# qingpingmo/OCN

Measured on AMD Instinct MI355X. Metric: candidate-edges/sec (CN predictor fwd), ogbl-collab shape, higher is better.
Workload: dtype f32

## Files before the change

include/ocn_hip.h:

```cpp
#ifndef OCN_HIP_H
#define OCN_HIP_H

#include <stdint.h>

#ifdef __cplusplus
extern "C" {
#endif

#define OCN_ABI_VERSION 9
#define OCN_EINVAL (-1)
#define OCN_ECAP   (-2)

#define OCN_ST_CAP  1
#define OCN_ST_SCAN 2
#define OCN_SCAN_POISON (-1)

#define OCN_F_CN1 1u
#define OCN_F_CN2 2u

int ocn_abi_version(void);

int64_t ocn_scan_workspace_bytes(int64_t n);

int ocn_zero_regions(void* const* ptrs, const int64_t* bytes, int32_t n, void* stream);
// ... 170 lines not shown
int ocn_philox4x32(const uint32_t* ctr , uint32_t key0, uint32_t key1, int64_t n, uint32_t* out ,
                   void* stream);
int ocn_complement_count(const int64_t* rowptrK, const int32_t* colK, int64_t n_cols, int32_t* count ,
                         void* stream);
int32_t ocn_sample_stage_cols(void);
int ocn_sample_complement_rows(const int64_t* rowptrK, const int32_t* colK, int64_t n_cols, const int64_t* rows, int64_t Q,
                               int64_t per, int64_t q0, uint64_t seed, int64_t* out , void* stream);
int ocn_sample_complement_pairs(const int64_t* rowptrK, const int32_t* colK, int64_t n_cols,
                                const int64_t* cptr , int64_t T, int64_t t0, uint64_t seed,
                                int64_t* out , void* stream);

int64_t ocn_sample_two_hop_window_cols(void);
int ocn_sample_two_hop(const int64_t* rowptrA, const int32_t* colA, const int64_t* rowptrM, const int32_t* colM, int64_t n_cols,
                       const int64_t* rows, int64_t Q, int32_t drop_self, int64_t window_cols ,
                       const int64_t* sptr , const int64_t* sid , int64_t q0, uint64_t seed,
                       int32_t* count , int64_t* out , void* stream);

int ocn_gather_schedule(const int32_t* gcost, int64_t n_groups, int64_t segment, int32_t* perm, void* stream);

int ocn_cn_weights_cn6(uint64_t* histA, uint64_t* histB, int64_t N, const float* innerprod, int32_t* scalars,
                       float* nip_out, const float* s2_exact , const float* s3_exact ,
                       void* stream);
int ocn_cn_gather3(const int64_t* rowptrA, const int32_t* colA, const int64_t* src, const int64_t* dst,
                   const int64_t* order, int64_t B, const int64_t* off, const uint8_t* flagsA,
                   const uint8_t* flagsB, const float* weightsA, const float* weightsB, const float* nip,
                   const float* h, int32_t H, float* xcn1, float* xcn2, float* xcn3, float* xij, void* stream);

int ocn_cn3_flags(const int64_t* rowptrA, const int32_t* colA, const int64_t* rowptrT, const int32_t* colT,
                  const uint32_t* bitmapP, int64_t bm_stride_words, const int64_t* src, const int64_t* dst,
                  const int64_t* order , int64_t B, int64_t n_cols, const int64_t* off, uint8_t* flags,
                  int64_t flags_cap, uint64_t* hist , int32_t* cnt3, int32_t* status,
                  const int64_t* nds , const int64_t* chunk_off , void* stream);

int ocn_cn_gather3_backward(const int64_t* rowptrA, const int32_t* colA, const int64_t* src, const int64_t* dst,
                            const int64_t* order, int64_t B, const int64_t* off, const uint8_t* flagsA,
                            const uint8_t* flagsB, const float* weightsA, const float* weightsB, const float* nip,
                            const float* h, int32_t H, const float* g1, const float* g2, const float* g3,
                            const float* g4, float* dh, void* stream);

int ocn_cn_gather_backward(const int64_t* rowptrA, const int32_t* colA,
                           const int64_t* src, const int64_t* dst, const int64_t* order, int64_t B,
                           const int64_t* off, const uint8_t* flags, const int32_t* wc,
                           const float* weights, const float* h, int32_t H,
                           const float* g1, const float* g2, const float* g3, float* dh, void* stream);

int64_t ocn_cn_gather_backward_det_workspace_bytes(int64_t N, int64_t B, int64_t flags_cap);
int ocn_cn_gather_backward_det(const int64_t* rowptrA, const int32_t* colA, const int64_t* src, const int64_t* dst,
                               int64_t B, const int64_t* off, const uint8_t* flags, const int32_t* wc, int64_t flags_cap,
                               const float* weights, const float* h, int64_t N, int32_t H, const float* g1,
                               const float* g2, const float* g3, float* dh, void* workspace, void* stream);
int64_t ocn_cn_gather_backward_det_keys_offset(int64_t N);
int ocn_cn_gather_backward_det_lists(const int64_t* rowptrA, const int32_t* colA, const int64_t* src, const int64_t* dst,
                                     int64_t B, const int64_t* off, const uint8_t* flags, int64_t flags_cap, int64_t N,
                                     void* workspace, void* stream);

int ocn_spmm_csr(const int64_t* rowptr, const int32_t* col, const float* val, int64_t n_rows,
                 const float* x, int32_t F, const float* pre, const float* post,
                 int32_t mode, int32_t edge_scale, int32_t self_mode,
                 float* y, void* stream);

int ocn_spmm_csr_rows(const int64_t* rowptr, const int32_t* col, const float* val, int64_t n_rows,
                      const float* x, int32_t F, const float* pre, const float* post,
                      int32_t mode, int32_t edge_scale, int32_t self_mode,
                      const int64_t* rows, int64_t n_list, float* y, void* stream);

int ocn_spmm_csr_max_arg(const int64_t* rowptr, const int32_t* col, const float* val, int64_t n_rows,
                         const float* x, int32_t F, float* y, int32_t* arg, void* stream);
int ocn_spmm_max_backward(const int64_t* rowptrT, const int32_t* colT, const float* valT, int64_t n_rows,
                          const int32_t* arg, const float* g, int32_t F, float* gx, void* stream);

int ocn_deg_rsqrt(const int64_t* rowptr, const float* val, int64_t n_rows, float add, float* out,
                  void* stream);

int64_t ocn_spgemm_max_cols(void);
int ocn_spgemm_pattern_count(const int64_t* rowptrA, const int32_t* colA, int64_t n_rows,
                             const int64_t* rowptrB, const int32_t* colB, int64_t n_colsB,
                             int32_t* row_count, uint32_t* bitmap ,
                             int64_t bm_stride_words, void* stream);
int ocn_spgemm_pattern_fill(const int64_t* rowptrA, const int32_t* colA, int64_t n_rows,
                            const int64_t* rowptrB, const int32_t* colB, int64_t n_colsB,
                            const int64_t* rowptrC, int32_t* colC, void* stream);
int32_t ocn_cn_flags_small_graph_cols(void);
int64_t ocn_cn_flags_pair_min_batch(int64_t min_rows);
int ocn_spgemm_bit_rows(const int64_t* rowptrA, const int32_t* colA, int64_t n_rows, const int64_t* rowptrB, const int32_t* colB,
                        int64_t n_colsB, const int64_t* rows, int64_t n_req, int32_t* done, uint32_t* bitmap,
                        int64_t bm_stride_words, void* stream);

int ocn_dense_from_csr(const int64_t* rowptr, const int32_t* col, int64_t n, int64_t ld, int8_t* dense, int8_t* denseT,
                       void* stream);
int ocn_dense_block_mm_bits(const int8_t* A, const int8_t* Bt, int64_t ld, int64_t K, int32_t r0, int32_t r1, int32_t c0,
                            int32_t c1, int32_t fold, uint32_t* bits, int64_t bm_stride_words, void* stream);
int ocn_bitrows_from_csr(const int64_t* rowptr, const int32_t* col, int64_t n_rows, uint32_t* bits, int64_t bm_stride_words,
                         void* stream);
int ocn_bitrows_count(const uint32_t* bits, int64_t bm_stride_words, int64_t n_rows, int64_t n_cols, int32_t* row_count,
                      void* stream);
int ocn_bitrows_fill(const uint32_t* bits, int64_t bm_stride_words, int64_t n_rows, int64_t n_cols, const int64_t* rowptr,
                     int32_t* col, void* stream);

int ocn_csr_union_count(const int64_t* rowptrA, const int32_t* colA, const int64_t* rowptrB, const int32_t* colB,
                        int64_t n_rows, int32_t* count, void* stream);
int ocn_csr_union_fill(const int64_t* rowptrA, const int32_t* colA, const int64_t* rowptrB, const int32_t* colB,
                       int64_t n_rows, const int64_t* rowptrC , int32_t* colC, void* stream);
int64_t ocn_bitrows_insert_workspace_bytes(int64_t nnzD);
int ocn_bitrows_insert(const int64_t* rowptrA, const int32_t* colA, const int64_t* rowptrT, const int32_t* colT,
                       const int64_t* rowptrD, const int32_t* colD, int64_t n, int64_t nnzD, uint32_t* bits,
                       int64_t bm_stride_words, int32_t* added, void* workspace, void* stream);

int ocn_csr_minus_count(const int64_t* rowptrA, const int32_t* colA, const int64_t* rowptrB, const int32_t* colB,
                        int64_t n_rows, int32_t* count, void* stream);
int ocn_csr_minus_fill(const int64_t* rowptrA, const int32_t* colA, const int64_t* rowptrB, const int32_t* colB,
                       int64_t n_rows, const int64_t* rowptrC , int32_t* colC, void* stream);
int64_t ocn_bitrows_remove_workspace_bytes(int64_t nnzD);
int ocn_bitrows_remove(const int64_t* rowptrA0, const int32_t* colA0, const int64_t* rowptrT0, const int32_t* colT0,
                       const int64_t* rowptrA, const int32_t* colA, const int64_t* rowptrT, const int32_t* colT,
                       const int64_t* rowptrD, const int32_t* colD, int64_t n, int64_t nnzD, uint32_t* bits,
                       int64_t bm_stride_words, int32_t* removed, void* workspace, void* stream);

int64_t ocn_rows_neighbourhood_workspace_bytes(int64_t n_list);
int ocn_rows_neighbourhood(const int64_t* rowptrT, const int32_t* colT, int64_t n, const int64_t* rows, int64_t n_list,
                           uint32_t* bits, void* workspace, void* stream);
int ocn_bitlist_count(const uint32_t* bits, int64_t n_bits, int32_t* count, void* stream);
int ocn_bitlist_fill(const uint32_t* bits, int64_t n_bits, const int64_t* off , int64_t* out,
                     void* stream);

int ocn_rows_ln_relu(const float* x, const float* gamma, const float* beta, float eps, int32_t relu,
                     int64_t rows, int32_t H, float* y, void* stream);
int ocn_combine3(const float* coef, const float* x1, const float* x2, const float* x3, int64_t n,
                 float* out, void* stream);

int ocn_fill_rows(float* dst, int64_t ld, int32_t n_cols, const float* vec, const int64_t* row_range,
                  int64_t max_rows, void* stream);

typedef struct OcnLinearGroup {
  const float* X; int64_t ldX;
  int64_t M;
  const void* Wp;
  const float* bias;
  const float* gamma; const float* beta; float eps;
  int32_t relu;
  const float* scale;
  const float* addend; int64_t ldAdd;
  const float* dotw; const float* dotb;
  float* Y; int64_t ldY;
  const int64_t* row_range;
  const int64_t* y_row_map;
  int32_t add_bcast;
} OcnLinearGroup;

int64_t ocn_linear_panel_bytes(int32_t N, int32_t K);
int ocn_linear_split_weight(const float* W, int32_t N, int32_t K, void* Wp, void* stream);
int ocn_linear_bf16x6(const float* X, int64_t M, int32_t K, const void* Wp, int32_t N,
                      const float* bias, const float* gamma, const float* beta, float eps,
                      int32_t relu, const float* dotw, const float* dotb, float* Y, void* stream);
int ocn_linear_grouped(const OcnLinearGroup* groups, int32_t n_groups, int32_t K, int32_t N, void* stream);

typedef struct OcnHeadsArgs {
  const float* x[3];
  int64_t ldx, B;
  int32_t H;
  const void* p_first[3];
  const void* p_mid[2];
  const void* p_out[3];
  const float* vec;
  const int64_t* ranges;
  const int64_t* y_row_map;
  float* y;
// ... 42 lines not shown
```

ocn_amd/_lib.py:

```python
from __future__ import annotations

import ctypes
import glob
import os
import subprocess
from ctypes import c_float, c_int32, c_int64, c_void_p

_HERE = os.path.dirname(os.path.abspath(__file__))
_ROOT = os.path.dirname(_HERE)
LIB_PATH = os.environ.get("OCN_LIB_PATH", os.path.join(_HERE, "libocn_hip.so"))
CSRC = os.path.join(_HERE, "csrc")
INCLUDE = os.path.join(_ROOT, "include")

_P = c_void_p
ABI_VERSION = 9
SIGNATURES = {
    "ocn_abi_version": (c_int32, []),
    "ocn_scan_workspace_bytes": (c_int64, [c_int64]),
    "ocn_zero_regions": (c_int32, [_P, _P, c_int32, _P]),
    "ocn_check_edges": (c_int32, [_P, _P, c_int64, c_int64, c_int64, _P, _P]),
    "ocn_edge_offsets": (c_int32, [_P, _P, c_int64, _P, _P, _P]),
    "ocn_class_order": (c_int32, [_P, _P, _P, c_int64, _P, _P, _P, _P, _P, _P]),
    "ocn_scan_i32": (c_int32, [_P, c_int64, _P, _P, _P]),
    "ocn_order_workspace_bytes": (c_int64, [c_int64]),
    "ocn_order_by_node": (c_int32, [_P, c_int64, c_int64, _P, _P, _P]),
    "ocn_order_by_node_finish": (c_int32, [_P, c_int64, c_int64, _P, _P, _P]),
    "ocn_order_by_node_finish_rec": (c_int32, [_P, _P, _P, _P, c_int64, c_int64, _P, _P, _P, _P]),
    "ocn_batch_prep": (c_int32, [_P, _P, c_int64, _P, _P, c_int64, _P, _P, _P, c_int32, _P]),
    "ocn_cn_flags": (c_int32, [_P, _P, _P, _P, _P, _P, _P, c_int64, _P, c_int64, _P, _P, _P, c_int64, c_int64, _P, _P, c_int64, _P,
                               _P, _P, _P, _P, _P, _P]),
    "ocn_cn_flags_rec": (c_int32, [_P, _P, _P, _P, _P, _P, _P, c_int64, _P, c_int64, _P, _P, _P, c_int64, c_int64, _P, _P, c_int64, _P,
                                   _P, _P, _P, _P, _P, _P]),
    "ocn_chunk_offsets": (c_int32, [_P, _P, _P, _P, c_int64, _P, _P, _P]),
    "ocn_walk_chunk": (c_int32, []),
    "ocn_cn_walk_flags": (c_int32, [_P, _P, _P, _P, _P, _P, c_int64, _P, _P, _P, c_int64, _P, _P, c_int64, _P, _P, _P,
                                    _P, _P]),
    "ocn_neighbor_degree_sum": (c_int32, [_P, _P, c_int64, _P, _P]),
    "ocn_walk_prep_max_batch": (c_int32, []),
    "ocn_cn_flags_small_graph_cols": (c_int32, []),
    "ocn_cn_flags_pair_min_batch": (c_int64, [c_int64]),
    "ocn_walk_prep": (c_int32, [_P, _P, _P, _P, c_int64, c_int32, _P, _P, _P, _P, _P, _P, _P, _P, _P, _P, _P, _P, _P]),
    "ocn_cn_walk_group": (c_int32, [_P, _P, _P, _P, _P, c_int64, _P, _P, _P, _P, _P, _P, _P, c_int64, _P, _P, _P, _P]),
    "ocn_walk_rev_offsets": (c_int32, [_P, _P, _P, _P, _P, c_int64, _P, _P, _P]),
    "ocn_cn_weights_cn5": (c_int32, [_P, c_int64, _P, _P, c_int32, _P, _P]),
    "ocn_cn5_column_stats": (c_int32, [_P, c_int64, _P, _P]),
    "ocn_cn_colsum_workspace_bytes": (c_int64, [c_int64, c_int64]),
    "ocn_cn_colsum_exact": (c_int32, [_P, _P, _P, c_int64, _P, _P, _P, _P, c_int64, _P, c_int64, _P, _P, _P, _P, _P, _P, _P]),
    "ocn_cn_weights_cn7": (c_int32, [_P, c_int64, c_float, _P, _P, _P]),
    "ocn_cn_gather": (c_int32, [_P, _P, _P, _P, _P, c_int64, _P, _P, _P, _P, _P, c_int32, c_int64, _P, _P, _P, _P, _P,
                                _P, _P, _P, _P, _P]),
    "ocn_cn8_pool": (c_int32, [_P, _P, _P, _P, _P, _P, _P, c_int64, _P, c_int64, _P, _P, _P, c_int64, c_int64, _P, c_int32, _P, _P,
                               _P, _P, _P, _P]),
    "ocn_cn_pool_frozen": (c_int32, [_P, _P, _P, _P, _P, _P, _P, c_int64, _P, c_int64, _P, _P, _P, c_int64, c_int64, _P, _P, c_int32, _P,
                                     _P, _P, _P, _P, _P]),
    "ocn_cn_attribution": (c_int32, [_P, _P, _P, _P, c_int64, _P, _P, _P, c_int64, _P, _P, c_int32, _P, _P, _P, _P, _P]),
    "ocn_cn_node_sums": (c_int32, [_P, _P, _P, _P, _P, _P, _P, c_int64, _P, c_int64, _P, _P, _P, c_int64, c_int64, _P, _P, _P, _P, _P,
                                   _P, _P]),
    "ocn_row_diff_stage_cols": (c_int32, []),
    "ocn_row_diff_count": (c_int32, [_P, _P, _P, _P, _P, c_int64, c_int32, _P, _P]),
    "ocn_row_diff_fill": (c_int32, [_P, _P, _P, _P, _P, c_int64, c_int32, _P, _P, _P]),
    "ocn_two_hop_window_cols": (c_int64, []),
    "ocn_two_hop_diff_count": (c_int32, [_P, _P, _P, _P, c_int64, _P, c_int64, c_int32, c_int64, _P, _P]),
    "ocn_two_hop_diff_fill": (c_int32, [_P, _P, _P, _P, c_int64, _P, c_int64, c_int32, c_int64, _P, _P, _P]),
    "ocn_two_hop_sums_window_cols": (c_int64, []),
    "ocn_two_hop_sums_fill": (c_int32, [_P, _P, _P, _P, c_int64, _P, c_int64, c_int32, c_int64, _P, c_int32, _P, _P, _P, _P]),
    "ocn_frontier_window_cols": (c_int64, []),
    "ocn_frontier_count": (c_int32, [_P, _P, _P, _P, c_int64, _P, c_int64, c_int32, c_int64, _P, _P, _P, _P, _P, _P]),
    "ocn_frontier_sums_fill": (c_int32, [_P, _P, _P, _P, c_int64, _P, c_int64, c_int32, c_int64, _P, _P, _P, _P, _P, _P, _P, _P, _P,
                                         _P]),
    "ocn_segment_topk_max_k": (c_int32, []),
    "ocn_segment_topk": (c_int32, [_P, _P, c_int64, c_int32, _P, _P, _P]),
    "ocn_segment_rank": (c_int32, [_P, _P, _P, c_int64, _P, _P, c_int64, _P, _P, _P]),
    "ocn_philox4x32": (c_int32, [_P, ctypes.c_uint32, ctypes.c_uint32, c_int64, _P, _P]),
    "ocn_complement_count": (c_int32, [_P, _P, c_int64, _P, _P]),
    "ocn_sample_stage_cols": (c_int32, []),
    "ocn_sample_complement_rows": (c_int32, [_P, _P, c_int64, _P, c_int64, c_int64, c_int64, ctypes.c_uint64, _P, _P]),
    "ocn_sample_complement_pairs": (c_int32, [_P, _P, c_int64, _P, c_int64, c_int64, ctypes.c_uint64, _P, _P]),
    "ocn_sample_two_hop_window_cols": (c_int64, []),
    "ocn_sample_two_hop": (c_int32, [_P, _P, _P, _P, c_int64, _P, c_int64, c_int32, c_int64, _P, _P, c_int64, ctypes.c_uint64, _P, _P,
                                     _P]),
    "ocn_gather_schedule": (c_int32, [_P, c_int64, c_int64, _P, _P]),
    "ocn_coo_to_csr_workspace_bytes": (c_int64, [c_int64, c_int64, c_int32, c_int32]),
    "ocn_coo_to_csr": (c_int32, [_P, _P, c_int64, c_int64, c_int64, c_int32, c_int32, _P, _P, _P, _P, _P]),
    "ocn_wgrad_workspace_bytes": (c_int64, [c_int64, c_int32, c_int32]),
    "ocn_wgrad": (c_int32, [_P, c_int64, _P, c_int64, c_int64, c_int32, c_int32, _P, _P, _P, _P]),
    "ocn_cn_weights_cn6": (c_int32, [_P, _P, c_int64, _P, _P, _P, _P, _P, _P]),
    "ocn_cn_gather3": (c_int32, [_P, _P, _P, _P, _P, c_int64, _P, _P, _P, _P, _P, _P, _P, c_int32, _P, _P, _P, _P, _P]),
    "ocn_cn3_flags": (c_int32, [_P, _P, _P, _P, _P, c_int64, _P, _P, _P, c_int64, c_int64, _P, _P, c_int64, _P, _P, _P, _P, _P, _P]),
    "ocn_cn_gather3_backward": (c_int32, [_P, _P, _P, _P, _P, c_int64, _P, _P, _P, _P, _P, _P, _P, c_int32, _P, _P, _P, _P, _P, _P]),
    "ocn_cn_gather_backward": (c_int32, [_P, _P, _P, _P, _P, c_int64, _P, _P, _P, _P, _P, c_int32, _P, _P, _P, _P, _P]),
    "ocn_cn_gather_backward_det_workspace_bytes": (c_int64, [c_int64, c_int64, c_int64]),
    "ocn_cn_gather_backward_det": (c_int32, [_P, _P, _P, _P, c_int64, _P, _P, _P, c_int64, _P, _P, c_int64, c_int32, _P, _P, _P, _P,
                                             _P, _P]),
    "ocn_cn_gather_backward_det_keys_offset": (c_int64, [c_int64]),
    "ocn_cn_gather_backward_det_lists": (c_int32, [_P, _P, _P, _P, c_int64, _P, _P, c_int64, c_int64, _P, _P]),
    "ocn_ln_drop_relu_workspace_bytes": (c_int64, [c_int32]),
    "ocn_ln_drop_relu_forward": (c_int32, [_P, _P, _P, c_float, c_float, ctypes.c_uint64, c_int32, c_int64, c_int32, _P, _P, _P]),
    "ocn_ln_drop_relu_backward": (c_int32, [_P, _P, _P, _P, _P, c_float, ctypes.c_uint64, c_int32, c_int64, c_int32, _P, _P, _P, _P, _P]),
    "ocn_dropout_keep_mask": (c_int32, [ctypes.c_uint64, c_float, c_int64, _P, _P]),
    "ocn_mix3_workspace_bytes": (c_int64, []),
    "ocn_mix3_backward": (c_int32, [_P, _P, _P, _P, _P, c_int64, _P, _P, _P, _P, _P, _P]),
    "ocn_spmm_csr": (c_int32, [_P, _P, _P, c_int64, _P, c_int32, _P, _P, c_int32, c_int32, c_int32, _P, _P]),
    "ocn_spmm_csr_rows": (c_int32, [_P, _P, _P, c_int64, _P, c_int32, _P, _P, c_int32, c_int32, c_int32, _P, c_int64, _P, _P]),
    "ocn_spmm_csr_max_arg": (c_int32, [_P, _P, _P, c_int64, _P, c_int32, _P, _P, _P]),
    "ocn_spmm_max_backward": (c_int32, [_P, _P, _P, c_int64, _P, _P, c_int32, _P, _P]),
    "ocn_deg_rsqrt": (c_int32, [_P, _P, c_int64, c_float, _P, _P]),
    "ocn_spgemm_max_cols": (c_int64, []),
    "ocn_spgemm_pattern_count": (c_int32, [_P, _P, c_int64, _P, _P, c_int64, _P, _P, c_int64, _P]),
    "ocn_spgemm_pattern_fill": (c_int32, [_P, _P, c_int64, _P, _P, c_int64, _P, _P, _P]),
    "ocn_spgemm_bit_rows": (c_int32, [_P, _P, c_int64, _P, _P, c_int64, _P, c_int64, _P, _P, c_int64, _P]),
    "ocn_dense_from_csr": (c_int32, [_P, _P, c_int64, c_int64, _P, _P, _P]),
    "ocn_dense_block_mm_bits": (c_int32, [_P, _P, c_int64, c_int64, c_int32, c_int32, c_int32, c_int32, c_int32, _P, c_int64, _P]),
    "ocn_bitrows_from_csr": (c_int32, [_P, _P, c_int64, _P, c_int64, _P]),
    "ocn_bitrows_count": (c_int32, [_P, c_int64, c_int64, c_int64, _P, _P]),
    "ocn_bitrows_fill": (c_int32, [_P, c_int64, c_int64, c_int64, _P, _P, _P]),
    "ocn_csr_union_count": (c_int32, [_P, _P, _P, _P, c_int64, _P, _P]),
    "ocn_csr_union_fill": (c_int32, [_P, _P, _P, _P, c_int64, _P, _P, _P]),
    "ocn_bitrows_insert_workspace_bytes": (c_int64, [c_int64]),
    "ocn_bitrows_insert": (c_int32, [_P, _P, _P, _P, _P, _P, c_int64, c_int64, _P, c_int64, _P, _P, _P]),
    "ocn_csr_minus_count": (c_int32, [_P, _P, _P, _P, c_int64, _P, _P]),
    "ocn_csr_minus_fill": (c_int32, [_P, _P, _P, _P, c_int64, _P, _P, _P]),
    "ocn_bitrows_remove_workspace_bytes": (c_int64, [c_int64]),
    "ocn_bitrows_remove": (c_int32, [_P, _P, _P, _P, _P, _P, _P, _P, _P, _P, c_int64, c_int64, _P, c_int64, _P, _P, _P]),
# ... 124 lines not shown
```

ocn_amd/csrc/cn_flags.hip:

```cpp
#include "common.h"


__device__ __forceinline__ bool sampled_has(const int32_t* samp, const int32_t* __restrict__ row, i64 n,
                                            int32_t key) {
  int lo = 0, hi = OCN_WAVE;
  while (lo < hi) {
    const int mid = (lo + hi) >> 1;
    if (samp[mid] <= key) lo = mid + 1; else hi = mid;
  }
  if (lo == 0) return false;
  const int s = lo - 1;
  const i64 p0 = ((i64)s * n) >> 6, p1 = ((i64)(s + 1) * n) >> 6;
  return sorted_has(row + p0, p1 - p0, key);
}

#define T1_CAP 1024

#define LH_MAX_COLS 8192

__device__ __forceinline__ i64 wave_uniform(i64 v) {
  const unsigned lo = __builtin_amdgcn_readfirstlane((unsigned)(u64)v), hi = __builtin_amdgcn_readfirstlane((unsigned)((u64)v >> 32));
  return (i64)(((u64)hi << 32) | lo);
}
__device__ __forceinline__ bool lanes_have(int32_t t, int32_t key) {
  int pos = 0;
#pragma unroll
  for (int step = OCN_WAVE / 2; step > 0; step >>= 1)
    if (__shfl(t, pos + step - 1, OCN_WAVE) < key) pos += step;
  return __shfl(t, pos, OCN_WAVE) == key;
}

template <bool HAS_T2, bool LH, bool RECIN, int NS>
__global__ __launch_bounds__(OCN_BLOCK) void cn_flags_kernel(
    const i64* __restrict__ rowptrA, const int32_t* __restrict__ colA,
    const i64* __restrict__ rowptrT1, const int32_t* __restrict__ colT1,
    const i64* __restrict__ rowptrT2, const int32_t* __restrict__ colT2,
    const unsigned* __restrict__ bmT1, i64 bm1_stride, const unsigned* __restrict__ bmT2, i64 bm_stride,
    const i64* __restrict__ src, const i64* __restrict__ dst, const i64* __restrict__ order, i64 B,
    i64 n_cols, const i64* __restrict__ off, uint8_t* __restrict__ flags, i64 cap,
    u64* __restrict__ hist, int32_t* __restrict__ cnt1, int32_t* __restrict__ cnt2,
    int32_t* __restrict__ status, u64* rec, int32_t* __restrict__ gcost) {
  constexpr int GPB = OCN_WPB, SPB = GPB * NS;
  constexpr int T1_PART = T1_CAP / NS, T2_PART = OCN_WAVE / NS;
  static_assert(NS == 1 || (NS == 2 && !LH), "slot pairs: large-graph forms only");
  __shared__ int s_cost[2][GPB];
  __shared__ int32_t s_t1[GPB][T1_CAP];
  __shared__ int32_t s_t2[GPB][OCN_WAVE];
  extern __shared__ __attribute__((aligned(16))) u64 s_hist[];
  const int gl = threadIdx.x % OCN_WAVE, g = __builtin_amdgcn_readfirstlane(threadIdx.x / OCN_WAVE);
  if (blockIdx.x == 0 && threadIdx.x == 0) status_raise(status, off[B], cap);
  const bool void_batch = off[B] < 0;
  if (LH) {
    for (i64 c = threadIdx.x; c < n_cols; c += OCN_BLOCK) s_hist[c] = 0ull;
    __syncthreads();
  }
  int par = 0;
  for (i64 e0 = (i64)blockIdx.x * SPB; e0 < B; e0 += (i64)gridDim.x * SPB, par ^= 1) {
    i64 slot[NS];
    bool act[NS];
    i64 e[NS], i[NS], j[NS], a0[NS], da[NS], b0[NS], db[NS], c0[NS], dc[NS], base[NS];
    const unsigned* bm_row[NS];
    const unsigned* bm1_row[NS];
#pragma unroll
    for (int s = 0; s < NS; ++s) {
      slot[s] = e0 + NS * g + s;
      act[s] = slot[s] < B;
      e[s] = i[s] = j[s] = a0[s] = da[s] = b0[s] = db[s] = c0[s] = dc[s] = base[s] = 0;
      bm_row[s] = bm1_row[s] = nullptr;
    }
    u64 recw = 0;
    if (RECIN && NS > 1 && gl < 4 * NS && slot[0] + gl / 4 < B) recw = rec[4 * slot[0] + gl];
#pragma unroll
    for (int s = 0; s < NS; ++s)
      if (act[s]) {
        if (RECIN) {
          u64 w[4];
          if (NS == 1) {
            const ulonglong2* rp = reinterpret_cast<const ulonglong2*>(rec + 4 * slot[s]);
            const ulonglong2 ra = rp[0], rb = rp[1];
            w[0] = ra.x; w[1] = ra.y; w[2] = rb.x; w[3] = rb.y;
          } else {
#pragma unroll
            for (int q = 0; q < 4; ++q)
              w[q] = (u64)(unsigned)__builtin_amdgcn_readlane((int)(unsigned)recw, 4 * s + q) |
                     ((u64)(unsigned)__builtin_amdgcn_readlane((int)(unsigned)(recw >> 32), 4 * s + q) << 32);
          }
          e[s] = wave_uniform((i64)w[0]);
          i[s] = wave_uniform((i64)(w[1] & 0xffffffffull)); j[s] = wave_uniform((i64)(w[1] >> 32));
          a0[s] = wave_uniform((i64)(w[2] & ((1ull << REC_LEN_SHIFT) - 1))); da[s] = wave_uniform((i64)(w[2] >> REC_LEN_SHIFT));
          base[s] = wave_uniform((i64)w[3]);
        } else {
          e[s] = order ? order[slot[s]] : slot[s];
          i[s] = src[e[s]]; j[s] = dst[e[s]];
          a0[s] = rowptrA[i[s]]; da[s] = rowptrA[i[s] + 1] - a0[s];
          base[s] = off[e[s]];
        }
        if (bmT1) bm1_row[s] = bmT1 + j[s] * bm1_stride;
        else { b0[s] = rowptrT1[j[s]]; db[s] = rowptrT1[j[s] + 1] - b0[s]; }
        if (HAS_T2) {
          if (bmT2) bm_row[s] = bmT2 + j[s] * bm_stride;
          if (rowptrT2 && (LH || !bmT2)) { c0[s] = rowptrT2[j[s]]; dc[s] = rowptrT2[j[s] + 1] - c0[s]; }
        }
        if (void_batch) { da[s] = 0; db[s] = 0; dc[s] = 0; base[s] = 0; }
      }
    bool t1_reg[NS], t1_lds[NS], t2_full[NS], t2_lds[NS];
    int t1_at[NS], t2_at[NS];
    int32_t t1[NS];
#pragma unroll
    for (int s = 0; s < NS; ++s) {
      const int o = (s + 1) % NS;
      const bool whole1 = NS == 1 || db[o] <= OCN_WAVE;
      t1_reg[s] = db[s] <= OCN_WAVE; t1_lds[s] = db[s] <= (whole1 ? T1_CAP : T1_PART);
      t1_at[s] = whole1 ? 0 : s * T1_PART;
      t1[s] = 0x7fffffff;
      if (t1_reg[s]) { if (gl < db[s]) t1[s] = colT1[b0[s] + gl]; }
      else if (t1_lds[s])
        for (i64 q = gl; q < db[s]; q += OCN_WAVE) s_t1[g][t1_at[s] + q] = colT1[b0[s] + q];
    }
#pragma unroll
    for (int s = 0; s < NS; ++s) {
      const int o = (s + 1) % NS;
      t2_full[s] = HAS_T2 && rowptrT2 && dc[s] == n_cols;
      const bool whole2 = NS == 1 || (HAS_T2 && rowptrT2 && dc[o] == n_cols) || dc[o] == 0;
      t2_lds[s] = whole2 || dc[s] <= T2_PART;
      t2_at[s] = whole2 ? 0 : s * T2_PART;
      if (HAS_T2 && !t2_full[s] && !bmT2 && t2_lds[s]) {
        if (dc[s] > OCN_WAVE) s_t2[g][gl] = colT2[c0[s] + (((i64)gl * dc[s]) >> 6)];
        else if (gl < dc[s]) s_t2[g][t2_at[s] + gl] = colT2[c0[s] + gl];
      }
    }
    wave_lds_sync();
    bool fits[NS];
    int c1[NS], c2[NS];
    i64 da_max = da[0];
#pragma unroll
    for (int s = 0; s < NS; ++s) {
      fits[s] = base[s] + da[s] <= cap;
      c1[s] = c2[s] = 0;
      if (s > 0 && da[s] > da_max) da_max = da[s];
    }
    const bool same = NS > 1 && i[0] == i[NS - 1];
    for (i64 p0 = 0; p0 < da_max; p0 += OCN_WAVE) {
      const i64 p = p0 + gl;
      bool in[NS], f1[NS], f2[NS];
      int32_t k[NS];
      unsigned w2[NS];
#pragma unroll
      for (int s = 0; s < NS; ++s) {
        in[s] = p < da[s];
        if (s > 0 && same) k[s] = k[0];
        else k[s] = in[s] ? colA[a0[s] + p] : 0;
      }
#pragma unroll
      for (int s = 0; s < NS; ++s) {
        w2[s] = 0;
        if (HAS_T2 && bmT2 && !t2_full[s] && in[s]) w2[s] = bm_row[s][k[s] >> 5];
      }
#pragma unroll
      for (int s = 0; s < NS; ++s) {
        if (bmT1) f1[s] = in[s] && ((bm1_row[s][k[s] >> 5] >> (k[s] & 31)) & 1u);
        else if (t1_reg[s]) f1[s] = lanes_have(t1[s], k[s]) && in[s];
        else f1[s] = in[s] && (t1_lds[s] ? sorted_has(&s_t1[g][t1_at[s]], db[s], k[s]) : sorted_has(colT1 + b0[s], db[s], k[s]));
      }
#pragma unroll
      for (int s = 0; s < NS; ++s) {
        f2[s] = false;
        if (HAS_T2 && in[s]) {
          if (t2_full[s]) f2[s] = true;
          else if (bmT2) f2[s] = (w2[s] >> (k[s] & 31)) & 1u;
          else if (!t2_lds[s]) f2[s] = sorted_has(colT2 + c0[s], dc[s], k[s]);
          else f2[s] = dc[s] > OCN_WAVE ? sampled_has(&s_t2[g][0], colT2 + c0[s], dc[s], k[s]) : sorted_has(&s_t2[g][t2_at[s]], dc[s], k[s]);
        }
        if (fits[s] && in[s]) flags[base[s] + p] = (uint8_t)((f1[s] ? OCN_F_CN1 : 0u) | (f2[s] ? OCN_F_CN2 : 0u));
      }
      if (NS > 1 && same) {
        u64 inc = 0;
#pragma unroll
        for (int s = 0; s < NS; ++s) inc += (u64)f1[s] | ((u64)f2[s] << HF_BITS) | ((u64)(f1[s] | f2[s]) << (2 * HF_BITS));
        if (inc) atomicAdd(hist + 2 * (i64)k[0], inc);
      } else {
#pragma unroll
        for (int s = 0; s < NS; ++s)
          if (f1[s] | f2[s]) {
            const u64 inc = (u64)f1[s] | ((u64)f2[s] << HF_BITS) | (1ull << (2 * HF_BITS));
            if (LH) atomicAdd(s_hist + k[s], inc); else atomicAdd(hist + 2 * (i64)k[s], inc);
          }
      }
#pragma unroll
      for (int s = 0; s < NS; ++s) {
        c1[s] += __popcll(__ballot(f1[s]));
        c2[s] += __popcll(__ballot(f2[s]));
      }
    }
    wave_lds_sync();
#pragma unroll
    for (int s = 0; s < NS; ++s)
      if (act[s] && gl == 0) {
        cnt1[e[s]] = c1[s];
        if (cnt2) cnt2[e[s]] = c2[s];
        if (rec) {
          u64* r = rec + 4 * slot[s];
          if (!RECIN) {
            r[0] = (u64)e[s];
            r[1] = (u64)i[s] | ((u64)j[s] << 32);
          }
          if (!RECIN || void_batch) r[2] = (u64)a0[s] | ((u64)da[s] << REC_LEN_SHIFT);
          r[3] = (u64)base[s] | ((u64)(da[s] > 0 && (i64)c2[s] == da[s]) << REC_FULL2_BIT) | ((u64)(c1[s] > 0) << 62) | ((u64)(c2[s] > 0) << 63);
        }
      }
    if (gcost) {
      int cost = act[0] ? c1[0] + c2[0] : 0;
#pragma unroll
      for (int s = 1; s < NS; ++s) cost = SCHED_COST(cost, act[s] ? c1[s] + c2[s] : 0);
      if (gl == 0) s_cost[par][g] = cost;
      __syncthreads();
      if (threadIdx.x == 0) {
#pragma unroll
        for (int q = 0; q < NS; ++q)
          if (NS == 1 || e0 + q * SCHED_GROUP < B) {
            int t = 0;
#pragma unroll
            for (int w = 0; w < GPB / NS; ++w) t = SCHED_COST(t, s_cost[par][q * (GPB / NS) + w]);
            gcost[e0 / SCHED_GROUP + q] = t;
          }
      }
    }
  }
  if (LH) {
    __syncthreads();
    for (i64 c = threadIdx.x; c < n_cols; c += OCN_BLOCK) {
      const u64 v = s_hist[c];
      if (v) atomicAdd(hist + 2 * c, v);
    }
  }
}

extern "C" {

int32_t ocn_cn_flags_small_graph_cols(void) { return LH_MAX_COLS; }

static int64_t g_flags_pair_min_batch = 32768;

int64_t ocn_cn_flags_pair_min_batch(int64_t min_rows) {
  const int64_t prev = g_flags_pair_min_batch;
  if (min_rows >= 0) g_flags_pair_min_batch = min_rows;
  return prev;
}

static int cn_flags_launch(const int64_t* rowptrA, const int32_t* colA, const int64_t* rowptrT1,
                           const int32_t* colT1, const int64_t* rowptrT2, const int32_t* colT2,
                           const uint32_t* bitmapT1, int64_t bm1_stride_words, const uint32_t* bitmapT2, int64_t bm_stride_words,
                           const int64_t* src, const int64_t* dst, const int64_t* order, int64_t B,
                           int64_t n_cols, const int64_t* off, uint8_t* flags, int64_t flags_cap, uint64_t* hist,
                           int32_t* cnt1, int32_t* cnt2, int32_t* status, uint64_t* rec, int32_t* gcost, bool rec_in, void* stream) {
  if (B < 0 || flags_cap < 0 || B > (int64_t)HF_MASK) return OCN_EINVAL;
  if (B == 0) return 0;
  if (!rowptrA || (!rowptrT1 && !bitmapT1) || !src || !dst || !off || !hist || !cnt1 || !status) return OCN_EINVAL;
  if (rec_in && (!rec || !order)) return OCN_EINVAL;
  if ((bitmapT1 && bm1_stride_words * 32 < n_cols) || (bitmapT2 && bm_stride_words * 32 < n_cols)) return OCN_EINVAL;
  constexpr int GPB = OCN_WPB;
  hipStream_t st = (hipStream_t)stream;
  const bool lh = n_cols > 0 && n_cols <= LH_MAX_COLS;
  const size_t lds = lh ? (size_t)n_cols * sizeof(u64) : 0;
  const bool pairs = !lh && B >= g_flags_pair_min_batch;
  const int spb = pairs ? 2 * GPB : GPB;
  const int grid = lh ? grid_for((B + GPB - 1) / GPB, 256 * 3) : grid_for((B + spb - 1) / spb);
  if (lh) {
    static bool raised_dev[64] = {};
    int devid = 0;
    if (hipGetDevice(&devid) != hipSuccess || devid < 0 || devid >= 64) return OCN_EINVAL;
    bool& raised = raised_dev[devid];
    if (!raised) {
      const void* fns[4] = {(const void*)cn_flags_kernel<true, true, false, 1>, (const void*)cn_flags_kernel<false, true, false, 1>,
                            (const void*)cn_flags_kernel<true, true, true, 1>, (const void*)cn_flags_kernel<false, true, true, 1>};
      for (const void* fn : fns) {
        hipError_t e1 = hipFuncSetAttribute(fn, hipFuncAttributeMaxDynamicSharedMemorySize, LH_MAX_COLS * (int)sizeof(u64));
        if (e1 != hipSuccess) return (int)e1;
      }
      raised = true;
    }
  }
#define CN_FLAGS_ARGS(T2P, T2C)                                                                      \
  (const i64*)rowptrA, colA, (const i64*)rowptrT1, colT1, (const i64*)(T2P), (T2C),                   \
      (const unsigned*)bitmapT1, (i64)bm1_stride_words, (const unsigned*)bitmapT2, (i64)bm_stride_words, (const i64*)src, \
      (const i64*)dst, (const i64*)order, (i64)B, (i64)n_cols, (const i64*)off, flags, (i64)flags_cap, \
      (u64*)hist, cnt1, cnt2, status, (u64*)rec, gcost
#define CN_FLAGS_LAUNCH(T2, LHV, RI, NSV, T2P, T2C)                                                   \
  hipLaunchKernelGGL((cn_flags_kernel<T2, LHV, RI, NSV>), dim3(grid), dim3(OCN_BLOCK), (LHV) ? lds : 0, st, CN_FLAGS_ARGS(T2P, T2C))
#define CN_FLAGS_PICK(T2, T2P, T2C)                                                                   \
  do {                                                                                                \
    if (lh) { if (rec_in) CN_FLAGS_LAUNCH(T2, true, true, 1, T2P, T2C); else CN_FLAGS_LAUNCH(T2, true, false, 1, T2P, T2C); }   \
    else if (pairs) { if (rec_in) CN_FLAGS_LAUNCH(T2, false, true, 2, T2P, T2C); else CN_FLAGS_LAUNCH(T2, false, false, 2, T2P, T2C); }   \
    else { if (rec_in) CN_FLAGS_LAUNCH(T2, false, true, 1, T2P, T2C); else CN_FLAGS_LAUNCH(T2, false, false, 1, T2P, T2C); }    \
  } while (0)
  if (!rowptrT2 && bitmapT2 && lh) return OCN_EINVAL;
  if (rowptrT2 || bitmapT2) CN_FLAGS_PICK(true, rowptrT2, colT2);
  else CN_FLAGS_PICK(false, nullptr, (const int32_t*)nullptr);
#undef CN_FLAGS_PICK
#undef CN_FLAGS_LAUNCH
  return launch_status();
}

int ocn_cn_flags(const int64_t* rowptrA, const int32_t* colA, const int64_t* rowptrT1,
                 const int32_t* colT1, const int64_t* rowptrT2, const int32_t* colT2,
                 const uint32_t* bitmapT1, int64_t bm1_stride_words, const uint32_t* bitmapT2, int64_t bm_stride_words,
                 const int64_t* src, const int64_t* dst, const int64_t* order, int64_t B,
                 int64_t n_cols, const int64_t* off, uint8_t* flags, int64_t flags_cap, uint64_t* hist,
                 int32_t* cnt1, int32_t* cnt2, int32_t* status, uint64_t* rec, int32_t* gcost, void* stream) {
  return cn_flags_launch(rowptrA, colA, rowptrT1, colT1, rowptrT2, colT2, bitmapT1, bm1_stride_words, bitmapT2, bm_stride_words,
                         src, dst, order, B, n_cols, off, flags, flags_cap, hist, cnt1, cnt2, status, rec, gcost, false, stream);
}

int ocn_cn_flags_rec(const int64_t* rowptrA, const int32_t* colA, const int64_t* rowptrT1,
                     const int32_t* colT1, const int64_t* rowptrT2, const int32_t* colT2,
                     const uint32_t* bitmapT1, int64_t bm1_stride_words, const uint32_t* bitmapT2, int64_t bm_stride_words,
                     const int64_t* src, const int64_t* dst, const int64_t* order, int64_t B,
                     int64_t n_cols, const int64_t* off, uint8_t* flags, int64_t flags_cap, uint64_t* hist,
                     int32_t* cnt1, int32_t* cnt2, int32_t* status, uint64_t* rec, int32_t* gcost, void* stream) {
  return cn_flags_launch(rowptrA, colA, rowptrT1, colT1, rowptrT2, colT2, bitmapT1, bm1_stride_words, bitmapT2, bm_stride_words,
                         src, dst, order, B, n_cols, off, flags, flags_cap, hist, cnt1, cnt2, status, rec, gcost, true, stream);
}

}
```

ocn_amd/ops.py:

```python
from __future__ import annotations

import ctypes
import os
from typing import Optional, Tuple

import torch
from torch import Tensor

from . import _lib
from ._lib import check, ptr, stream_ptr

FLAGS_NOSYNC_LIMIT = 1 << 30
validate_indices = True
stage_timer = None
LN_WIDTHS = (16, 32, 64, 128, 256, 512)
a1_bitmap_max_bytes = int(os.environ.get("OCN_A1_BITMAP_MAX_BYTES", 64 << 20))
a2_bitmap_max_bytes = 16 << 30
skip_zero_rows = True
skip_zero_min_share = 0.15
skip_zero_backoff = 32
skip_zero_min_batch = 4096
walk_two_sided = True
walk_share_min = 2
sort_edges_min_batch = 4096
# ... 1528 lines not shown
def mix3_backward(coef: Tensor, g: Tensor, x1: Tensor, x2: Tensor, x3: Tensor):
    g = _req(g.contiguous(), torch.float32, "g")
    for t, nm in ((x1, "x1"), (x2, "x2"), (x3, "x3")):
        if _req(t, torch.float32, nm).shape != g.shape:
            raise ValueError("mix3_backward: shape mismatch")
    n = g.numel()
    if n % 4:
        raise ValueError("mix3_backward: n must be a multiple of 4")
    l = _lib.lib()
    d1, d2, d3 = torch.empty_like(g), torch.empty_like(g), torch.empty_like(g)
    dcoef = torch.empty(3, dtype=torch.float32, device=g.device)
    ws = torch.empty(int(l.ocn_mix3_workspace_bytes()), dtype=torch.uint8, device=g.device)
    check(l.ocn_mix3_backward(ptr(coef), ptr(g), ptr(x1), ptr(x2), ptr(x3), n, ptr(d1), ptr(d2), ptr(d3), ptr(dcoef), ptr(ws),
                              stream_ptr()), "ocn_mix3_backward")
    return d1, d2, d3, dcoef


@_on_device
def fill_rows(dst: Tensor, vec: Tensor, row_range: Tensor) -> None:
    _req_strided(dst, "dst")
    _req(vec, torch.float32, "vec")
    _req(row_range, torch.int64, "row_range", 1)
    if vec.numel() != dst.shape[1]:
        raise ValueError("fill_rows: width mismatch")
    check(_lib.lib().ocn_fill_rows(ptr(dst), dst.stride(0), dst.shape[1], ptr(vec), ptr(row_range), dst.shape[0],
                                   stream_ptr()), "ocn_fill_rows")
    _mark("mlp_glue")


LINEAR_WIDTHS = (32, 64, 128, 256)
fast_linear = True
_panels: dict = {}


@_on_device
def linear_panel(weight: Tensor) -> Tensor:
    import weakref
    key = id(weight)
    hit = _panels.get(key)
    if (hit is not None and hit[0]() is weight and hit[1] == weight.data_ptr() and hit[2] == weight._version
            and hit[3] == tuple(weight.shape)):
        return hit[4]
    w = _req(weight.detach(), torch.float32, "weight", 2)
    N, K = w.shape
    panel = torch.empty(int(_lib.lib().ocn_linear_panel_bytes(N, K)), dtype=torch.uint8, device=w.device)
    check(_lib.lib().ocn_linear_split_weight(ptr(w), N, K, ptr(panel), stream_ptr()), "ocn_linear_split_weight")
    if len(_panels) > 512:
        for k in [k for k, v in _panels.items() if v[0]() is None]:
            del _panels[k]
    _panels[key] = (weakref.ref(weight), weight.data_ptr(), weight._version, (N, K), panel)
    return panel


@_on_device
def heads_panel(weight: Tensor):
    import math
    w = _req(weight.detach(), torch.float32, "weight", 2)
    N, K = w.shape
    m = float(w.abs().max().item()) if w.numel() else 0.0
    if not math.isfinite(m):
        raise ValueError("heads_panel: non-finite weight")
    sw = 13 - math.frexp(m)[1] + 1 if m > 0.0 else 0
    sw = max(-100, min(100, sw))
    panel = torch.empty(int(_lib.lib().ocn_heads_panel_bytes(N, K)), dtype=torch.uint8, device=w.device)
    check(_lib.lib().ocn_heads_split_weight(ptr(w), N, K, float(2.0 ** sw), ptr(panel), stream_ptr()), "ocn_heads_split_weight")
    return panel, float(2.0 ** -sw)


HEADS_WIDTHS = (128, 256)
train_linear = True
train_tails = os.environ.get("OCN_TRAIN_TAILS", "1") != "0"
fused_heads = True
fused_heads_min_width = 128


def heads_small_batch(max_rows: int = -1) -> int:
    return int(_lib.lib().ocn_heads_small_batch(int(max_rows)))


def flags_pair_min_batch(min_rows: int = -1) -> int:
    return int(_lib.lib().ocn_cn_flags_pair_min_batch(int(min_rows)))


@_on_device
def heads_fused(x1: Tensor, x2: Tensor, xij: Tensor, pack: dict, ranges: Optional[Tensor], y_row_map: Optional[Tensor],
                b_on_union: bool, scratch: Tensor, dump: Optional[Tensor] = None) -> Optional[Tensor]:
    for t, nm in ((x1, "xcn1"), (x2, "xcn2"), (xij, "xij")):
        _req(t, torch.float32, nm, 2)
    B, H = xij.shape
    if x1.shape != (B, H) or x2.shape != (B, H) or H not in HEADS_WIDTHS:
        raise ValueError("heads_fused: shape mismatch")
    a = _lib.OcnHeadsArgs()
    a.x[0], a.x[1], a.x[2] = x1.data_ptr(), x2.data_ptr(), xij.data_ptr()
    a.ldx, a.B, a.H = H, B, H
    for i in range(3):
        a.p_first[i] = pack["first"][i].data_ptr()
        a.p_out[i] = pack["out"][i].data_ptr()
    a.p_mid[0], a.p_mid[1] = pack["mid"][0].data_ptr(), pack["mid"][1].data_ptr()
    a.vec = pack["vec"].data_ptr()
    a.ranges = 0 if ranges is None else _req(ranges, torch.int64, "ranges").data_ptr()
    a.y_row_map = 0 if y_row_map is None else _req(y_row_map, torch.int64, "y_row_map", 1).data_ptr()
    y = None
    nconst = int(_lib.lib().ocn_heads_const_bytes(H)) // 4
    if dump is None:
        y = torch.empty((B, 1), dtype=torch.float32, device=xij.device)
        a.y = y.data_ptr()
        if _req(pack["cpark"], torch.float32, "cpark", 1).numel() != nconst:
            raise ValueError("heads_fused: constants buffer of the wrong size")
        a.cpark = pack["cpark"].data_ptr()
    else:
        if B != 1 or _req(dump, torch.float32, "dump", 1).numel() != nconst:
            raise ValueError("heads_fused: constants mode takes one row and ocn_heads_const_bytes(H) bytes")
        a.dump = dump.data_ptr()
    if scratch.numel() * scratch.element_size() < int(_lib.lib().ocn_heads_scratch_bytes(H)):
        raise ValueError("heads_fused: scratch too small")
    a.scratch = scratch.data_ptr()
    a.eps, a.ln, a.b_on_union = float(pack["eps"]), int(pack["ln"]), int(bool(b_on_union))
    _mark("mlp_glue")
    check(_lib.lib().ocn_heads_fused(ctypes.byref(a), stream_ptr()), "ocn_heads_fused")
    _mark("linear", pack["flops_per_row"] * B)
    return y


def linear_ok(x: Tensor, weight: Tensor) -> bool:
    return (fast_linear and x.is_cuda and x.dim() == 2 and x.dtype == torch.float32 and x.is_contiguous()
            and weight.shape[0] in LINEAR_WIDTHS and weight.shape[1] % 16 == 0 and weight.shape[1] == x.shape[1])


@_on_device
def linear(x: Tensor, weight: Tensor, bias: Optional[Tensor] = None, ln=None, relu: bool = False,
           dot=None, y_row_map: Optional[Tensor] = None) -> Tensor:
    _req(x, torch.float32, "x", 2)
    M, K = x.shape
    N = weight.shape[0]
    if y_row_map is not None:
        if dot is None:
            raise ValueError("y_row_map needs the dot epilogue")
        y = torch.empty((M, 1), dtype=torch.float32, device=x.device)
        linear_grouped([dict(x=x, weight=weight, bias=bias, ln=ln, relu=relu, dot=(dot[0].reshape(1, -1), dot[1]), y=y,
                             y_row_map=y_row_map)], K, N)
        return y
    panel = linear_panel(weight)
    _mark("mlp_glue")
    y = torch.empty((M, 1) if dot is not None else (M, N), dtype=torch.float32, device=x.device)
    g = b = None
    eps = 0.0
    if ln is not None:
        g, b, eps = ln
    dw = db = None
    if dot is not None:
        dw, db = dot
        dw = dw.reshape(-1)
    check(_lib.lib().ocn_linear_bf16x6(ptr(x), M, K, ptr(panel), N, ptr(bias), ptr(g), ptr(b), float(eps),
                                       int(relu), ptr(dw), ptr(db), ptr(y), stream_ptr()), "ocn_linear_bf16x6")
    _mark("linear", 2.0 * M * K * N)
    return y


def linear_ok_t(gy: Tensor, weight: Tensor) -> bool:
    return (fast_linear and gy.is_cuda and gy.dim() == 2 and gy.dtype == torch.float32
            and weight.shape[1] in LINEAR_WIDTHS and weight.shape[0] % 16 == 0 and weight.shape[0] == gy.shape[1])


@_on_device
def linear_t(gy: Tensor, weight: Tensor) -> Tensor:
    gy = _req(gy.contiguous(), torch.float32, "gy", 2)
# ... 117 lines not shown
```

Before: 177.6 million.

## Add four-slots-per-wave cn_flags variant and narrow per-slot index types

Generalizes the cn_flags kernel from one or two edge slots per wave to four. Slot-sharing logic for T1/T2 staging, same-row reuse and histogram merging now works across any number of slots, and when a wave owns a whole schedule group it writes gcost directly instead of going through LDS and __syncthreads. Per-slot indices and lengths are narrowed from 64-bit to 32-bit to cut register use. The quad path is gated by a batch threshold that defaults to 2^40, so only the type narrowing and generalized loops reach default runs; the quad variant adds register pressure and extra template instantiations.

```diff
diff --git a/include/ocn_hip.h b/include/ocn_hip.h
--- a/include/ocn_hip.h
+++ b/include/ocn_hip.h
@@ -276,6 +276,7 @@
                             const int64_t* rowptrC, int32_t* colC, void* stream);
 int32_t ocn_cn_flags_small_graph_cols(void);
 int64_t ocn_cn_flags_pair_min_batch(int64_t min_rows);
+int64_t ocn_cn_flags_quad_min_batch(int64_t min_rows);
 int ocn_spgemm_bit_rows(const int64_t* rowptrA, const int32_t* colA, int64_t n_rows, const int64_t* rowptrB, const int32_t* colB,
                         int64_t n_colsB, const int64_t* rows, int64_t n_req, int32_t* done, uint32_t* bitmap,
                         int64_t bm_stride_words, void* stream);
diff --git a/ocn_amd/_lib.py b/ocn_amd/_lib.py
--- a/ocn_amd/_lib.py
+++ b/ocn_amd/_lib.py
@@ -39,6 +39,7 @@
     "ocn_walk_prep_max_batch": (c_int32, []),
     "ocn_cn_flags_small_graph_cols": (c_int32, []),
     "ocn_cn_flags_pair_min_batch": (c_int64, [c_int64]),
+    "ocn_cn_flags_quad_min_batch": (c_int64, [c_int64]),
     "ocn_walk_prep": (c_int32, [_P, _P, _P, _P, c_int64, c_int32, _P, _P, _P, _P, _P, _P, _P, _P, _P, _P, _P, _P, _P]),
     "ocn_cn_walk_group": (c_int32, [_P, _P, _P, _P, _P, c_int64, _P, _P, _P, _P, _P, _P, _P, c_int64, _P, _P, _P, _P]),
     "ocn_walk_rev_offsets": (c_int32, [_P, _P, _P, _P, _P, c_int64, _P, _P, _P]),
diff --git a/ocn_amd/csrc/cn_flags.hip b/ocn_amd/csrc/cn_flags.hip
--- a/ocn_amd/csrc/cn_flags.hip
+++ b/ocn_amd/csrc/cn_flags.hip
@@ -22,6 +22,7 @@
   const unsigned lo = __builtin_amdgcn_readfirstlane((unsigned)(u64)v), hi = __builtin_amdgcn_readfirstlane((unsigned)((u64)v >> 32));
   return (i64)(((u64)hi << 32) | lo);
 }
+__device__ __forceinline__ unsigned wave_uniform(unsigned v) { return __builtin_amdgcn_readfirstlane(v); }
 __device__ __forceinline__ bool lanes_have(int32_t t, int32_t key) {
   int pos = 0;
 #pragma unroll
@@ -42,7 +43,9 @@
     int32_t* __restrict__ status, u64* rec, int32_t* __restrict__ gcost) {
   constexpr int GPB = OCN_WPB, SPB = GPB * NS;
   constexpr int T1_PART = T1_CAP / NS, T2_PART = OCN_WAVE / NS;
-  static_assert(NS == 1 || (NS == 2 && !LH), "slot pairs: large-graph forms only");
+  constexpr bool OWN_GROUP = NS == SCHED_GROUP;
+  static_assert(NS == 1 || ((NS == 2 || NS == 4) && !LH), "several slots per wave: large-graph forms only");
+  static_assert(GPB % NS == 0 && SPB % SCHED_GROUP == 0, "a workgroup is whole schedule groups of whole waves");
   __shared__ int s_cost[2][GPB];
   __shared__ int32_t s_t1[GPB][T1_CAP];
   __shared__ int32_t s_t2[GPB][OCN_WAVE];
@@ -58,7 +61,9 @@
   for (i64 e0 = (i64)blockIdx.x * SPB; e0 < B; e0 += (i64)gridDim.x * SPB, par ^= 1) {
     i64 slot[NS];
     bool act[NS];
-    i64 e[NS], i[NS], j[NS], a0[NS], da[NS], b0[NS], db[NS], c0[NS], dc[NS], base[NS];
+    i64 a0[NS], b0[NS], c0[NS], base[NS];
+    int e[NS], da[NS], db[NS], dc[NS];
+    unsigned i[NS], j[NS];
     const unsigned* bm_row[NS];
     const unsigned* bm1_row[NS];
 #pragma unroll
@@ -85,21 +90,21 @@
               w[q] = (u64)(unsigned)__builtin_amdgcn_readlane((int)(unsigned)recw, 4 * s + q) |
                      ((u64)(unsigned)__builtin_amdgcn_readlane((int)(unsigned)(recw >> 32), 4 * s + q) << 32);
           }
-          e[s] = wave_uniform((i64)w[0]);
-          i[s] = wave_uniform((i64)(w[1] & 0xffffffffull)); j[s] = wave_uniform((i64)(w[1] >> 32));
-          a0[s] = wave_uniform((i64)(w[2] & ((1ull << REC_LEN_SHIFT) - 1))); da[s] = wave_uniform((i64)(w[2] >> REC_LEN_SHIFT));
+          e[s] = (int)wave_uniform((unsigned)w[0]);
+          i[s] = wave_uniform((unsigned)w[1]); j[s] = wave_uniform((unsigned)(w[1] >> 32));
+          a0[s] = wave_uniform((i64)(w[2] & ((1ull << REC_LEN_SHIFT) - 1))); da[s] = (int)wave_uniform((unsigned)(w[2] >> REC_LEN_SHIFT));
           base[s] = wave_uniform((i64)w[3]);
         } else {
-          e[s] = order ? order[slot[s]] : slot[s];
-          i[s] = src[e[s]]; j[s] = dst[e[s]];
-          a0[s] = rowptrA[i[s]]; da[s] = rowptrA[i[s] + 1] - a0[s];
+          e[s] = (int)(order ? order[slot[s]] : slot[s]);
+          i[s] = (unsigned)src[e[s]]; j[s] = (unsigned)dst[e[s]];
+          a0[s] = rowptrA[i[s]]; da[s] = (int)(rowptrA[(i64)i[s] + 1] - a0[s]);
           base[s] = off[e[s]];
         }
         if (bmT1) bm1_row[s] = bmT1 + j[s] * bm1_stride;
-        else { b0[s] = rowptrT1[j[s]]; db[s] = rowptrT1[j[s] + 1] - b0[s]; }
+        else { b0[s] = rowptrT1[j[s]]; db[s] = (int)(rowptrT1[(i64)j[s] + 1] - b0[s]); }
         if (HAS_T2) {
           if (bmT2) bm_row[s] = bmT2 + j[s] * bm_stride;
-          if (rowptrT2 && (LH || !bmT2)) { c0[s] = rowptrT2[j[s]]; dc[s] = rowptrT2[j[s] + 1] - c0[s]; }
+          if (rowptrT2 && (LH || !bmT2)) { c0[s] = rowptrT2[j[s]]; dc[s] = (int)(rowptrT2[(i64)j[s] + 1] - c0[s]); }
         }
         if (void_batch) { da[s] = 0; db[s] = 0; dc[s] = 0; base[s] = 0; }
       }
@@ -108,8 +113,10 @@
     int32_t t1[NS];
 #pragma unroll
     for (int s = 0; s < NS; ++s) {
-      const int o = (s + 1) % NS;
-      const bool whole1 = NS == 1 || db[o] <= OCN_WAVE;
+      bool whole1 = true;
+#pragma unroll
+      for (int o = 0; o < NS; ++o)
+        if (o != s) whole1 = whole1 && db[o] <= OCN_WAVE;
       t1_reg[s] = db[s] <= OCN_WAVE; t1_lds[s] = db[s] <= (whole1 ? T1_CAP : T1_PART);
       t1_at[s] = whole1 ? 0 : s * T1_PART;
       t1[s] = 0x7fffffff;
@@ -119,9 +126,11 @@
     }
 #pragma unroll
     for (int s = 0; s < NS; ++s) {
-      const int o = (s + 1) % NS;
       t2_full[s] = HAS_T2 && rowptrT2 && dc[s] == n_cols;
-      const bool whole2 = NS == 1 || (HAS_T2 && rowptrT2 && dc[o] == n_cols) || dc[o] == 0;
+      bool whole2 = true;
+#pragma unroll
+      for (int o = 0; o < NS; ++o)
+        if (o != s) whole2 = whole2 && ((HAS_T2 && rowptrT2 && dc[o] == n_cols) || dc[o] == 0);
       t2_lds[s] = whole2 || dc[s] <= T2_PART;
       t2_at[s] = whole2 ? 0 : s * T2_PART;
       if (HAS_T2 && !t2_full[s] && !bmT2 && t2_lds[s]) {
@@ -132,23 +141,25 @@
     wave_lds_sync();
     bool fits[NS];
     int c1[NS], c2[NS];
-    i64 da_max = da[0];
+    int da_max = da[0];
 #pragma unroll
     for (int s = 0; s < NS; ++s) {
       fits[s] = base[s] + da[s] <= cap;
       c1[s] = c2[s] = 0;
       if (s > 0 && da[s] > da_max) da_max = da[s];
     }
-    const bool same = NS > 1 && i[0] == i[NS - 1];
-    for (i64 p0 = 0; p0 < da_max; p0 += OCN_WAVE) {
-      const i64 p = p0 + gl;
+    bool run[NS];
+#pragma unroll
+    for (int s = 0; s < NS; ++s) run[s] = s > 0 && i[s] == i[s - 1];
+    for (int p0 = 0; p0 < da_max; p0 += OCN_WAVE) {
+      const int p = p0 + gl;
       bool in[NS], f1[NS], f2[NS];
       int32_t k[NS];
       unsigned w2[NS];
 #pragma unroll
       for (int s = 0; s < NS; ++s) {
         in[s] = p < da[s];
-        if (s > 0 && same) k[s] = k[0];
+        if (s > 0 && run[s]) k[s] = k[s - 1];
         else k[s] = in[s] ? colA[a0[s] + p] : 0;
       }
 #pragma unroll
@@ -173,19 +184,17 @@
         }
         if (fits[s] && in[s]) flags[base[s] + p] = (uint8_t)((f1[s] ? OCN_F_CN1 : 0u) | (f2[s] ? OCN_F_CN2 : 0u));
       }
-      if (NS > 1 && same) {
-        u64 inc = 0;
-#pragma unroll
-        for (int s = 0; s < NS; ++s) inc += (u64)f1[s] | ((u64)f2[s] << HF_BITS) | ((u64)(f1[s] | f2[s]) << (2 * HF_BITS));
-        if (inc) atomicAdd(hist + 2 * (i64)k[0], inc);
-      } else {
-#pragma unroll
-        for (int s = 0; s < NS; ++s)
-          if (f1[s] | f2[s]) {
-            const u64 inc = (u64)f1[s] | ((u64)f2[s] << HF_BITS) | (1ull << (2 * HF_BITS));
-            if (LH) atomicAdd(s_hist + k[s], inc); else atomicAdd(hist + 2 * (i64)k[s], inc);
-          }
-      }
+      u64 inc[NS];
+#pragma unroll
+      for (int s = 0; s < NS; ++s) inc[s] = (u64)f1[s] | ((u64)f2[s] << HF_BITS) | ((u64)(f1[s] | f2[s]) << (2 * HF_BITS));
+#pragma unroll
+      for (int s = NS - 1; s > 0; --s)
+        if (run[s]) { inc[s - 1] += inc[s]; inc[s] = 0; }
+#pragma unroll
+      for (int s = 0; s < NS; ++s)
+        if (inc[s]) {
+          if (LH) atomicAdd(s_hist + k[s], inc[s]); else atomicAdd(hist + 2 * (i64)k[s], inc[s]);
+        }
 #pragma unroll
       for (int s = 0; s < NS; ++s) {
         c1[s] += __popcll(__ballot(f1[s]));
@@ -212,17 +221,21 @@
       int cost = act[0] ? c1[0] + c2[0] : 0;
 #pragma unroll
       for (int s = 1; s < NS; ++s) cost = SCHED_COST(cost, act[s] ? c1[s] + c2[s] : 0);
-      if (gl == 0) s_cost[par][g] = cost;
-      __syncthreads();
-      if (threadIdx.x == 0) {
-#pragma unroll
-        for (int q = 0; q < NS; ++q)
-          if (NS == 1 || e0 + q * SCHED_GROUP < B) {
-            int t = 0;
-#pragma unroll
-            for (int w = 0; w < GPB / NS; ++w) t = SCHED_COST(t, s_cost[par][q * (GPB / NS) + w]);
-            gcost[e0 / SCHED_GROUP + q] = t;
-          }
+      if constexpr (OWN_GROUP) {
+        if (act[0] && gl == 0) gcost[slot[0] / SCHED_GROUP] = cost;
+      } else {
+        if (gl == 0) s_cost[par][g] = cost;
+        __syncthreads();
+        if (threadIdx.x == 0) {
+#pragma unroll
+          for (int q = 0; q < NS; ++q)
+            if (NS == 1 || e0 + q * SCHED_GROUP < B) {
+              int t = 0;
+#pragma unroll
+              for (int w = 0; w < GPB / NS; ++w) t = SCHED_COST(t, s_cost[par][q * (GPB / NS) + w]);
+              gcost[e0 / SCHED_GROUP + q] = t;
+            }
+        }
       }
     }
   }
@@ -244,6 +257,14 @@
 int64_t ocn_cn_flags_pair_min_batch(int64_t min_rows) {
   const int64_t prev = g_flags_pair_min_batch;
   if (min_rows >= 0) g_flags_pair_min_batch = min_rows;
+  return prev;
+}
+
+static int64_t g_flags_quad_min_batch = (int64_t)1 << 40;
+
+int64_t ocn_cn_flags_quad_min_batch(int64_t min_rows) {
+  const int64_t prev = g_flags_quad_min_batch;
+  if (min_rows >= 0) g_flags_quad_min_batch = min_rows;
   return prev;
 }
 
@@ -263,7 +284,8 @@
   const bool lh = n_cols > 0 && n_cols <= LH_MAX_COLS;
   const size_t lds = lh ? (size_t)n_cols * sizeof(u64) : 0;
   const bool pairs = !lh && B >= g_flags_pair_min_batch;
-  const int spb = pairs ? 2 * GPB : GPB;
+  const bool quads = pairs && B >= g_flags_quad_min_batch;
+  const int spb = quads ? 4 * GPB : pairs ? 2 * GPB : GPB;
   const int grid = lh ? grid_for((B + GPB - 1) / GPB, 256 * 3) : grid_for((B + spb - 1) / spb);
   if (lh) {
     static bool raised_dev[64] = {};
@@ -290,6 +312,7 @@
 #define CN_FLAGS_PICK(T2, T2P, T2C)                                                                   \
   do {                                                                                                \
     if (lh) { if (rec_in) CN_FLAGS_LAUNCH(T2, true, true, 1, T2P, T2C); else CN_FLAGS_LAUNCH(T2, true, false, 1, T2P, T2C); }   \
+    else if (quads) { if (rec_in) CN_FLAGS_LAUNCH(T2, false, true, 4, T2P, T2C); else CN_FLAGS_LAUNCH(T2, false, false, 4, T2P, T2C); }   \
     else if (pairs) { if (rec_in) CN_FLAGS_LAUNCH(T2, false, true, 2, T2P, T2C); else CN_FLAGS_LAUNCH(T2, false, false, 2, T2P, T2C); }   \
     else { if (rec_in) CN_FLAGS_LAUNCH(T2, false, true, 1, T2P, T2C); else CN_FLAGS_LAUNCH(T2, false, false, 1, T2P, T2C); }    \
   } while (0)
diff --git a/ocn_amd/ops.py b/ocn_amd/ops.py
--- a/ocn_amd/ops.py
+++ b/ocn_amd/ops.py
@@ -1634,6 +1634,10 @@
     return int(_lib.lib().ocn_cn_flags_pair_min_batch(int(min_rows)))
 
 
+def flags_quad_min_batch(min_rows: int = -1) -> int:
+    return int(_lib.lib().ocn_cn_flags_quad_min_batch(int(min_rows)))
+
+
 @_on_device
 def heads_fused(x1: Tensor, x2: Tensor, xij: Tensor, pack: dict, ranges: Optional[Tensor], y_row_map: Optional[Tensor],
                 b_on_union: bool, scratch: Tensor, dump: Optional[Tensor] = None) -> Optional[Tensor]:
```

Result: no change. 178.2 million, median of 5 (+0.3%).
